# Farama-Foundation/Gymnasium

Hardware: AMD Instinct MI355X
Metric: env-steps/sec at num_envs=65536 (1/2/4/8 MI355X) vs CPU AsyncVectorEnv (higher is better)
Workload: dtype f64

## Files before the change

### gymnasium_amd/csrc/classic_kernels.h

```cpp
#ifndef MI355ENV_CLASSIC_KERNELS_H
#define MI355ENV_CLASSIC_KERNELS_H
#include "lane_step.h"
#include "wrappers_internal.h"

namespace {

MI_DEV double clip_to(double v, int flags, double lo, double hi) {
    if (flags & 1) v = v < lo ? lo : v;
    if (flags & 2) v = v > hi ? hi : v;
    return v;
}
__host__ __device__ inline bool epi_reduces(const EpiDev &e) { return (e.obs_on && e.obs_update) || (e.ret_on && e.ret_update); }

template <int NC>
MI_DEV void block_sum_columns(double (&v)[NC], double (*sh)[kEpiCols]) {
    const int wave = threadIdx.x >> 6, lane = threadIdx.x & 63;
#pragma unroll
    for (int k = 0; k < NC; k++) {
#pragma unroll
        for (int off = 32; off > 0; off >>= 1) v[k] += __shfl_xor(v[k], off, 64);
    }
    __syncthreads();
    if (lane == 0) {
#pragma unroll
        for (int k = 0; k < NC; k++) sh[wave][k] = v[k];
    }
    __syncthreads();
    if (threadIdx.x < NC) {
        double t = 0;
#pragma unroll
        for (int w = 0; w < kBlock / 64; w++) t += sh[w][threadIdx.x];
        v[0] = t;
    }
}

template <class E>
MI_DEV void epilogue_phase1(const EpiDev &e, int i, bool valid, const float *obs, double &reward, bool terminated) {
    constexpr int OBS = E::OBS, NC = 2 * OBS + 3;
    static_assert(OBS <= kEpiObsMax, "epilogue rows are sized for the classic-control observations");
    double v[NC];
#pragma unroll
    for (int k = 0; k < NC; k++) v[k] = 0;
    if (valid) {
        double r = clip_to(reward, e.clip_pre, e.pre_lo, e.pre_hi);
        if (e.ret_on) {
            const bool pd = e.prev_done[i] != 0, active = e.same_step || !pd;
            float a = e.acc[i];
            if (active) {
                const float g = a * e.gamma;
                a = (float)((double)g * (terminated ? 0.0 : 1.0) + r);
                e.acc[i] = a;
            }
            if (e.ret_update && active) {
                const double d = (double)a - e.ret_mean[0];
                v[2 * OBS] = d, v[2 * OBS + 1] = d * d, v[2 * OBS + 2] = 1.0;
            }
        } else {
            r = clip_to(r, e.clip_post, e.post_lo, e.post_hi);
        }
        reward = r;
        if (e.obs_on && e.obs_update) {
#pragma unroll
            for (int c = 0; c < OBS; c++) {
                const double d = (double)obs[c] - e.obs_mean[c];
                v[c] = d, v[OBS + c] = d * d;
            }
        }
    }
    if (!epi_reduces(e)) return;
    __shared__ double sh[kBlock / 64][kEpiCols];
    block_sum_columns<NC>(v, sh);
    if (threadIdx.x < NC) e.partial[(size_t)blockIdx.x * kEpiCols + threadIdx.x] = v[0];
}

template <int OBS>
MI_DEV void epilogue_statistics(const EpiDev &e, int N, bool fold, double (*sh)[kEpiCols], double *st) {
    constexpr int NC = 2 * OBS + 3;
    if (threadIdx.x < OBS && e.obs_on) st[threadIdx.x] = e.obs_mean[threadIdx.x], st[OBS + threadIdx.x] = e.obs_var[threadIdx.x];
    if (threadIdx.x == 64) {
        st[2 * OBS] = e.ret_on ? e.ret_var[0] : 1.0, st[2 * OBS + 1] = e.ret_on ? e.ret_mean[0] : 0.0;
        st[2 * OBS + 2] = e.obs_on ? *e.obs_count : 0.0, st[2 * OBS + 3] = e.ret_on ? *e.ret_count : 0.0;
    }
    if (fold) {
        double v[NC];
// ... 349 lines not shown
            ar.request(at, d, i);
            ar.arrive(L.trig);
        }
        u128 astate = 0;
        if (SAMPLE) {
            if (as.lane_valid) {
                astate = make_u128(as.lane[i], as.lane[(size_t)d.N + i]);
            } else {
                astate = make_u128(as.state_hi, as.state_lo);
                uint32_t delta = (uint32_t)i + 1u;
                for (int j = 0; delta; j++, delta >>= 1)
                    if (delta & 1u) astate = as.pow2[j].mult * astate + as.pow2[j].plus;
            }
        }
        const size_t N = (size_t)d.N;
        ResetQueue<E> q;
        q.have = 0u;
        q.rng = load_rng(d, i);
        WrapLaneOf<E, MAXSKIP> sl;
        load_wrap_lane(w, i, sl);
        if constexpr (MAXSKIP) load_skip_lane(w, d, i, sl);
        for (int t = 0; t < T; t++) {
            typename E::Act a;
            if (SAMPLE) {
                a = action_of_state<E>(astate);
                astate = as.jump_n.mult * astate + as.jump_n.plus;
                if (io.actions_out) static_cast<typename E::Act *>(io.actions_out)[t * N + i] = a;
            } else {
                a = static_cast<const typename E::Act *>(io.actions_in)[t * N + i];
            }
            StepOut<E> o;
            if (MODE == MI_AUTORESET_SAME_STEP) {
#pragma unroll
                for (int k = 0; k < E::OBS; k++) o.final_obs[k] = 0.0f;
            }
            if constexpr (MAXSKIP) q.have = 0u;
            lane_step_wrapped<E, MODE, MAXSKIP>(d, w, sl, i, L, a, o, st, &q, nullptr);
            if (io.obs) store_row<E::OBS>(static_cast<float *>(io.obs) + (t * N + i) * E::OBS, o.obs);
            if (io.reward) io.reward[t * N + i] = o.reward;
            if (io.terminated) io.terminated[t * N + i] = o.terminated;
            if (io.truncated) io.truncated[t * N + i] = o.truncated;
            if (ex.ep_ret) ex.ep_ret[t * N + i] = o.ep_ret;
            if (ex.ep_len) ex.ep_len[t * N + i] = o.ep_len;
            if (MODE == MI_AUTORESET_SAME_STEP && ex.final_obs) store_row<E::OBS>(static_cast<float *>(ex.final_obs) + (t * N + i) * E::OBS, o.final_obs);
        }
        if constexpr (MAXSKIP) {
            int wi = i;
            hold_opaque(wi);
            store_lane<E>(d, wi, L);
            store_wrap_lane(w, wi, sl);
            sl.written = 1u;
            store_skip_lane(w, d, wi, sl);
            store_rng_state(d, wi, q.rng);
            if (SAMPLE && as.lane) as.lane[wi] = (uint64_t)(astate >> 64), as.lane[N + wi] = (uint64_t)astate;
        } else {
            store_lane<E>(d, i, L);
            store_wrap_lane(w, i, sl);
            if (q.have) {
#pragma unroll
                for (int k = 0; k < E::NDRAWS; k++) q.rng.unstep();
            }
            store_rng_state(d, i, q.rng);
            if (SAMPLE && as.lane) as.lane[i] = (uint64_t)(astate >> 64), as.lane[N + i] = (uint64_t)astate;
        }
    }
    block_accumulate(d, st);
}

constexpr int kDuoBlock = 2 * kBlock;
template <class E>
struct DuoTraits {
#ifdef MI_DUO_CHUNK_OVERRIDE
    static constexpr int CHUNK = MI_DUO_CHUNK_OVERRIDE;
#else
    static constexpr int CHUNK = E::DUO_CHUNK;
#endif
};

template <class E, class = void>
struct HasRareHook : std::false_type {};
template <class E>
struct HasRareHook<E, std::void_t<decltype(E::RARE_HOOK)>> : std::integral_constant<bool, E::RARE_HOOK> {};

template <class E>
MI_DEV void duo_env_step(const DevEnv &d, Lane<E> &L, typename E::Act a, ResetQueue<E> &q, float obs[E::OBS], double &reward, uint32_t &bits) {
    const bool resetting = (L.flags & kNeedsReset) != 0;
    const bool refill = resetting && !q.have;
    constexpr bool HOOK = HasRareHook<E>::value && !E::SPLIT_TERMINAL && !E::AUX_REWARD;
    if (!HOOK && __builtin_expect(refill, 0)) q.refill();
    const double (&rs)[E::S] = q.rs;
    const uint32_t rflags = ResetQueue<E>::reset_flags(L.flags & ~kNeedsReset);
    double rew;
    bool te;
    uint32_t sflags = L.flags;
    if constexpr (E::SPLIT_TERMINAL) {
        E::integrate(L.s, sflags, a, L.trig);
#pragma unroll
        for (int k = 0; k < E::S; k++) L.s[k] = resetting ? rs[k] : L.s[k];
        E::obs(L.s, sflags, obs, L.trig);
        E::terminal_after_obs(L.s, L.trig, rew, te);
    } else if constexpr (E::AUX_REWARD) {
        E::advance(L.s, a, d.P, L.trig);
        rew = 0.0, te = false;
    } else if constexpr (HOOK) {
        E::step_hooked(L.s, sflags, a, d.P, rew, te, L.trig, refill, [&]() __attribute__((always_inline)) {
            if (refill) q.refill();
        });
    } else {
        E::step(L.s, sflags, a, d.P, rew, te, L.trig);
    }
    const uint32_t elapsed = L.elapsed + 1u;
    const bool tr = d.max_steps > 0 && (int)elapsed >= d.max_steps;
    const bool done = !resetting && (te || tr);
    if constexpr (!E::SPLIT_TERMINAL) {
#pragma unroll
        for (int k = 0; k < E::S; k++) L.s[k] = resetting ? rs[k] : L.s[k];
    }
    L.flags = resetting ? rflags : (done ? (sflags | kNeedsReset) : sflags);
    L.elapsed = resetting ? 0u : elapsed;
    q.have = resetting ? 0u : q.have;
    if constexpr (!E::SPLIT_TERMINAL) E::obs(L.s, L.flags, obs, L.trig);
    reward = resetting ? 0.0 : rew;
    bits = (resetting ? 4u : 0u) | ((!resetting && te) ? 1u : 0u) | ((!resetting && tr) ? 2u : 0u);
}

template <class E>
MI_DEV void duo_env_step_state(const DevEnv &d, Lane<E> &L, typename E::Act a, ResetQueue<E> &q, double *w64, float *w32) {
    static_assert(!E::SPLIT_TERMINAL, "the split terminal test belongs to the observation, which this role does not take");
    const bool resetting = (L.flags & kNeedsReset) != 0;
    if (__builtin_expect(resetting && !q.have, 0)) q.refill();
    const double (&rs)[E::S] = q.rs;
    const uint32_t rflags = ResetQueue<E>::reset_flags(L.flags & ~kNeedsReset);
    double rew;
    bool te;
    uint32_t sflags = L.flags;
    E::step(L.s, sflags, a, d.P, rew, te, L.trig);
    const uint32_t elapsed = L.elapsed + 1u;
    const bool tr = d.max_steps > 0 && (int)elapsed >= d.max_steps;
    const bool done = !resetting && (te || tr);
#pragma unroll
    for (int k = 0; k < E::S; k++) L.s[k] = resetting ? rs[k] : L.s[k];
    L.flags = resetting ? rflags : (done ? (sflags | kNeedsReset) : sflags);
    L.elapsed = resetting ? 0u : elapsed;
    q.have = resetting ? 0u : q.have;
    E::aux_pack(L.s, w64, w32);
}

template <class E>
__global__ __launch_bounds__(kDuoBlock) void rollout_duo_kernel(DevEnv d, RolloutPtrs io, ActionStream as, int T) {
    typedef typename E::Act Act;
    constexpr int ROLES = 2;
    constexpr int C = DuoTraits<E>::CHUNK;
    typedef Act ActLds;
    constexpr bool ACT_AHEAD = E::DUO_ACT_AHEAD;
    __shared__ ActLds sh_act[2][C + (ACT_AHEAD ? 1 : 0)][kBlock];
    constexpr bool DERIVE = E::AUX_DERIVES_FLAGS;
    static_assert(!DERIVE || E::REWARD_FROM_TERMINATED, "an aux role that derives the flags also derives the reward from them");
    constexpr int NF64 = E::AUX_F64 > 0 ? E::AUX_F64 : 1, NF32 = E::AUX_F32 > 0 ? E::AUX_F32 : 1;
    __shared__ double sh_w64[DERIVE ? 2 : 1][DERIVE ? C : 1][DERIVE ? kBlock : 1][NF64];
    __shared__ float sh_w32[(DERIVE && E::AUX_F32 > 0) ? 2 : 1][(DERIVE && E::AUX_F32 > 0) ? C : 1][(DERIVE && E::AUX_F32 > 0) ? kBlock : 1][NF32];
    __shared__ float sh_obs[DERIVE ? 1 : 2][DERIVE ? 1 : C][DERIVE ? 1 : kBlock][E::OBS];
    constexpr bool AUXREW = E::AUX_REWARD;
    constexpr bool REW_OF_ACT = E::AUX_REWARD_OF_ACTION;
    constexpr bool PASS_REWARD = !E::REWARD_FROM_TERMINATED && !AUXREW && !REW_OF_ACT;
    __shared__ double sh_pre[AUXREW ? 2 : 1][AUXREW ? C : 1][AUXREW ? kBlock : 1][E::AUX_PRE];
    __shared__ double sh_rew[PASS_REWARD ? 2 : 1][PASS_REWARD ? C : 1][kBlock];
    typedef typename std::conditional<E::REWARD_FROM_TERMINATED && E::OBS == 4, uint32_t, uint8_t>::type MI_DUO_FLAG_T;
    __shared__ MI_DUO_FLAG_T sh_bits[DERIVE ? 1 : 2][DERIVE ? 1 : C][DERIVE ? 1 : kBlock];
    __shared__ uint64_t sh_c[4][kBlock / 64];
    __shared__ double sh_r[kBlock / 64];
#ifdef MI_DUO_TIMING
    const unsigned long long t_begin = __builtin_readcyclecounter();
#endif
    tables_init<E>();
    const int role = threadIdx.x / kBlock;
    const bool is_env = role == 0, is_policy = role == 1, is_book = role == ROLES - 1;
    const int slot = threadIdx.x & (kBlock - 1);
    const int i = blockIdx.x * kBlock + slot;
    const bool active = i < d.N;
    const size_t N = (size_t)d.N;
    LaneStats st = {0u, 0u, 0u, 0ull, 0.0};
    Lane<E> L;
    ResetQueue<E> q;
    u128 astate = 0;
    double ep_ret = 0.0;
    int32_t ep_len = 0, ep_len_start = 0;
    uint32_t n_term = 0;
    uint32_t start_flags = 0;
    uint32_t aux_elapsed = 0, aux_needs_reset = 0;
    if (active) {
        if (is_env) {
            load_lane<E>(d, i, L);
            q.have = 0u;
            q.rng = load_rng(d, i);
        }
        if (is_book) {
            ep_ret = d.ep_ret[i], ep_len = d.ep_len[i];
            const uint32_t meta0 = d.meta[i];
            start_flags = meta0 >> kFlagShift;
            aux_elapsed = meta0 & kElapsedMask, aux_needs_reset = start_flags & kNeedsReset;
            ep_len_start = (start_flags & kNeedsReset) ? 0 : ep_len;
        }
        if (is_policy) {
            if (as.lane_valid) {
                astate = make_u128(as.lane[i], as.lane[N + i]);
            } else {
                astate = make_u128(as.state_hi, as.state_lo);
                uint32_t delta = (uint32_t)i + 1u;
                for (int j = 0; delta; j++, delta >>= 1)
                    if (delta & 1u) astate = as.pow2[j].mult * astate + as.pow2[j].plus;
            }
        }
    }
    const int chunks = T / C;
#ifdef MI_DUO_TIMING
    unsigned long long t_work = 0, t_wait = 0, t_wait0 = 0, t_mark = __builtin_readcyclecounter();
    const unsigned long long t_prologue = t_mark - t_begin;
#endif
    auto phase = [&](auto env_tag, const int p) __attribute__((always_inline)) {
        constexpr bool ENV = decltype(env_tag)::value;
        if (active) {
            if constexpr (ENV) {
                const int c = p - 1;
                if (c >= 0 && c < chunks) {
                    const int buf = c & 1;
                    constexpr bool REFILL_PER_CHUNK = kRefillPeriod % C == 0;
                    if (REFILL_PER_CHUNK && ((c * C) & (kRefillPeriod - 1)) == 0 && !q.have) q.refill();
                    ActLds a_next = sh_act[buf][0][slot];
#ifdef MI_DUO_ENV_UNROLL
#pragma unroll MI_DUO_ENV_UNROLL
#else
#pragma unroll 1
#endif
                    for (int k = 0; k < C; k++) {
                        const int t = c * C + k;
                        if (!REFILL_PER_CHUNK && (t & (kRefillPeriod - 1)) == 0 && !q.have) q.refill();
                        const Act a_k = ACT_AHEAD ? (Act)a_next : (Act)sh_act[buf][k][slot];
                        if (ACT_AHEAD) a_next = sh_act[buf][k + 1][slot];
                        if constexpr (DERIVE) {
                            double w64[NF64];
                            float w32[NF32];
                            duo_env_step_state<E>(d, L, a_k, q, w64, w32);
#pragma unroll
                            for (int j = 0; j < E::AUX_F64; j++) sh_w64[buf][k][slot][j] = w64[j];
#pragma unroll
                            for (int j = 0; j < E::AUX_F32; j++) sh_w32[buf][k][slot][j] = w32[j];
                        } else {
                            float o[E::OBS];
                            double rew;
                            uint32_t bits;
                            uint32_t pre_pending = 0u;
                            if constexpr (AUXREW) {
                                double pre[E::AUX_PRE];
                                pre_pending = E::aux_pre(L.s, pre);
#pragma unroll
                                for (int j = 0; j < E::AUX_PRE; j++) sh_pre[buf][k][slot][j] = pre[j];
                            }
                            duo_env_step<E>(d, L, a_k, q, o, rew, bits);
                            if constexpr (AUXREW && E::AUX_PRE_SQUARES > 0) bits |= pre_pending << 3;
#pragma unroll
                            for (int j = 0; j < E::OBS; j++) sh_obs[buf][k][slot][j] = o[j];
                            if constexpr (PASS_REWARD) sh_rew[buf][k][slot] = rew;
                            sh_bits[buf][k][slot] = (MI_DUO_FLAG_T)bits;
                        }
                    }
                }
            } else {
                const int c = p - 2;
                if (is_book && c >= 0) {
                    const int buf = c & 1;
                    if constexpr (AUXREW && E::AUX_PRE_SQUARES > 0) {
                        static_assert(E::AUX_PRE_SQUARES * C <= 32 && E::AUX_PRE_SQUARES <= 4 && sizeof(MI_DUO_FLAG_T) == 1, "pending bits: one word per chunk, bits 3 .. 6 of the flag byte");
                        uint32_t pend = 0u;
#pragma unroll
                        for (int k = 0; k < C; k++)
                            pend |= (((uint32_t)sh_bits[buf][k][slot] >> 3) & ((1u << E::AUX_PRE_SQUARES) - 1u)) << (E::AUX_PRE_SQUARES * k);
#pragma nounroll
                        while (pend) {
                            const int idx = __builtin_ctz(pend);
                            double *x = &sh_pre[buf][idx / E::AUX_PRE_SQUARES][slot][idx % E::AUX_PRE_SQUARES];
                            *x = E::aux_square(*x);
                            pend &= pend - 1u;
                        }
                    }
                    if constexpr (AUXREW) {
                        if constexpr (E::AUX_ACT_SQUARE) {
                            static_assert(C <= 32 && sizeof(ActLds) == sizeof(float), "one pending bit per step; the square takes the action's place");
                            uint32_t apend = 0u;
#pragma unroll
                            for (int k = 0; k < C; k++) {
                                const float u = E::act_square_arg((Act)sh_act[buf][k][slot]);
                                float h;
                                const bool plain = E::Math::sqf_is_plain(u, h);
                                sh_act[buf][k][slot] = (ActLds)(plain ? h : u);
                                apend |= plain ? 0u : 1u << k;
                            }
#pragma nounroll
                            while (apend) {
                                ActLds *x = &sh_act[buf][__builtin_ctz(apend)][slot];
                                *x = (ActLds)E::Math::sqf((float)*x);
                                apend &= apend - 1u;
                            }
                        }
                    }
#pragma unroll
                    for (int k = 0; k < C; k++) {
                        const size_t t = (size_t)c * C + k;
                        float o[E::OBS];
                        bool resetting, te, tr;
                        if constexpr (DERIVE) {
                            double w64[NF64];
                            float w32[NF32];
#pragma unroll
                            for (int j = 0; j < E::AUX_F64; j++) w64[j] = sh_w64[buf][k][slot][j];
#pragma unroll
                            for (int j = 0; j < E::AUX_F32; j++) w32[j] = sh_w32[buf][k][slot][j];
                            bool t0;
                            E::aux_unpack(w64, w32, d.P, o, t0);
                            resetting = aux_needs_reset != 0;
                            const uint32_t el = aux_elapsed + 1u;
                            te = !resetting && t0;
                            tr = !resetting && d.max_steps > 0 && (int)el >= d.max_steps;
                            aux_elapsed = resetting ? 0u : el;
                            aux_needs_reset = (te || tr) ? 1u : 0u;
                        } else {
#pragma unroll
                            for (int j = 0; j < E::OBS; j++) o[j] = sh_obs[buf][k][slot][j];
                            const uint32_t bits = sh_bits[buf][k][slot];
                            resetting = (bits & 4u) != 0, te = (bits & 1u) != 0, tr = (bits & 2u) != 0;
                        }
                        double rew;
                        const bool done = te || tr;
                        if constexpr (E::REWARD_FROM_TERMINATED) {
                            rew = resetting ? 0.0 : E::reward_from_terminated(te, d.P);
                            if constexpr (!DERIVE) ep_len = resetting ? 0 : ep_len + 1;
                            st.reset_steps += resetting ? 1u : 0u;
                            st.episodes += done ? 1u : 0u;
                            n_term += te ? 1u : 0u;
                        } else {
                            if constexpr (AUXREW) {
                                double pre[E::AUX_PRE];
#pragma unroll
                                for (int j = 0; j < E::AUX_PRE; j++) pre[j] = sh_pre[buf][k][slot][j];
                                if constexpr (E::AUX_ACT_SQUARE)
                                    rew = resetting ? 0.0 : E::aux_reward_squared(pre, (float)sh_act[buf][k][slot]);
                                else
                                    rew = resetting ? 0.0 : E::aux_reward(pre, (Act)sh_act[buf][k][slot]);
                            } else if constexpr (REW_OF_ACT) {
                                rew = resetting ? 0.0 : E::reward_of_action(te, (Act)sh_act[buf][k][slot]);
                            } else {
                                rew = sh_rew[buf][k][slot];
                            }
                            const double ret = ep_ret + rew;
                            const int32_t len = ep_len + 1;
                            ep_ret = resetting ? 0.0 : ret;
                            ep_len = resetting ? 0 : len;
                            st.reset_steps += resetting ? 1u : 0u;
                            st.env_steps += resetting ? 0u : 1u;
                            st.episodes += done ? 1u : 0u;
                            st.return_sum += done ? ret : 0.0;
                            st.length_sum += done ? (uint64_t)len : 0ull;
                        }
                        store_row<E::OBS>(static_cast<float *>(io.obs) + (t * N + i) * E::OBS, o);
                        io.reward[t * N + i] = rew;
                        io.terminated[t * N + i] = te;
                        io.truncated[t * N + i] = tr;
                    }
                }
                if (is_policy && p < chunks) {
                    const int buf = p & 1;
#pragma unroll
                    for (int k = 0; k < C; k++) {
                        const size_t t = (size_t)p * C + k;
                        const Act a = action_of_state<E>(astate);
                        astate = as.jump_n.mult * astate + as.jump_n.plus;
                        sh_act[buf][k][slot] = (ActLds)a;
                        static_cast<Act *>(io.actions_out)[t * N + i] = a;
                    }
                }
            }
        }
#ifdef MI_DUO_TIMING
        {
            const unsigned long long now = __builtin_readcyclecounter();
            t_work += now - t_mark, t_mark = now;
        }
#endif
        __syncthreads();
#ifdef MI_DUO_TIMING
        {
            const unsigned long long now = __builtin_readcyclecounter();
            if (p == 0) t_wait0 = now - t_mark;
            t_wait += now - t_mark, t_mark = now;
        }
#endif
    };
    if (__builtin_amdgcn_readfirstlane((int)is_env)) {
#pragma unroll 1
        for (int p = 0; p < chunks + 2; p++) phase(std::true_type(), p);
    } else {
#pragma unroll 1
        for (int p = 0; p < chunks + 2; p++) phase(std::false_type(), p);
    }
#ifdef MI_DUO_TIMING
    if (blockIdx.x == 7 && (threadIdx.x & 63) == 0)
        printf("duo timing: wave %d (role %d) prologue %llu work %llu wait-at-barrier %llu (phase 0: %llu) cycles over %d phases\n", (int)(threadIdx.x >> 6), role,
               t_prologue, t_work, t_wait, t_wait0, chunks + 2);
#endif
    if (active) {
        if (is_env) {
#pragma unroll
            for (int k = 0; k < E::S; k++) d.state[(size_t)k * d.N + i] = L.s[k];
            d.meta[i] = (L.elapsed & kElapsedMask) | (L.flags << kFlagShift);
            if (q.have) {
#pragma unroll
                for (int k = 0; k < E::NDRAWS; k++) q.rng.unstep();
            }
            store_rng_state(d, i, q.rng);
        } else if (is_book) {
            if constexpr (E::REWARD_FROM_TERMINATED) {
                const double r_n = E::reward_from_terminated(false, d.P), r_t = E::reward_from_terminated(true, d.P);
                bool last_done, last_te;
                if constexpr (DERIVE) {
                    double w64[NF64];
                    float w32[NF32], o[E::OBS];
#pragma unroll
                    for (int j = 0; j < E::AUX_F64; j++) w64[j] = sh_w64[((chunks > 0 ? chunks : 1) - 1) & 1][C - 1][slot][j];
#pragma unroll
                    for (int j = 0; j < E::AUX_F32; j++) w32[j] = sh_w32[((chunks > 0 ? chunks : 1) - 1) & 1][C - 1][slot][j];
                    bool t0;
                    E::aux_unpack(w64, w32, d.P, o, t0);
                    last_done = aux_needs_reset != 0, last_te = last_done && t0;
                } else {
                    const uint32_t last_bits = chunks > 0 ? (uint32_t)sh_bits[(chunks - 1) & 1][C - 1][slot] : ((start_flags & kNeedsReset) ? 2u : 0u);
                    last_done = (last_bits & 3u) != 0, last_te = (last_bits & 1u) != 0;
                }
                if (DERIVE && chunks > 0) ep_len = st.reset_steps ? (int32_t)aux_elapsed : ep_len + chunks * C;
                st.env_steps = (uint32_t)(chunks * C) - st.reset_steps;
                st.length_sum = (uint64_t)((int64_t)st.env_steps + (int64_t)ep_len_start - (last_done ? (int64_t)0 : (int64_t)ep_len));
                st.return_sum = r_n * (double)((int64_t)st.length_sum - (int64_t)n_term) + r_t * (double)n_term;
                st.return_sum = st.episodes ? st.return_sum : 0.0;
                ep_ret = (last_done && last_te) ? r_n * (double)(ep_len - 1) + r_t : r_n * (double)ep_len;
                if (chunks == 0) ep_ret = d.ep_ret[i];
            }
            d.ep_ret[i] = ep_ret, d.ep_len[i] = ep_len;
        }
        if (is_policy && as.lane) {
            int w = i;
            hold_opaque(w);
            as.lane[w] = (uint64_t)(astate >> 64), as.lane[N + w] = (uint64_t)astate;
        }
    }
    const int wave = slot >> 6, lane = threadIdx.x & 63;
    if (is_book) {
        const uint32_t c0 = wave_sum(st.env_steps), c1 = wave_sum(st.reset_steps), c2 = wave_sum(st.episodes);
        const uint64_t c3 = c2 ? wave_sum(st.length_sum) : 0;
        const double r = c2 ? wave_sum(st.return_sum) : 0.0;
        if (lane == 0) sh_c[0][wave] = c0, sh_c[1][wave] = c1, sh_c[2][wave] = c2, sh_c[3][wave] = c3, sh_r[wave] = r;
    }
    __syncthreads();
    if (threadIdx.x < 4) {
        uint64_t t = 0;
#pragma unroll
        for (int w = 0; w < kBlock / 64; w++) t += sh_c[threadIdx.x][w];
        if (t) d.blk_count[(size_t)blockIdx.x * 4 + threadIdx.x] += t;
    } else if (threadIdx.x == 64) {
        double t = 0.0;
#pragma unroll
        for (int w = 0; w < kBlock / 64; w++) t += sh_r[w];
        if (t != 0.0) d.blk_ret[blockIdx.x] += t;
    }
}

MI_DEV u128 shared_advance(const SharedRng &sr, u128 state, uint64_t n) {
    for (int j = 0; n; j++, n >>= 1)
        if (n & 1ull) state = sr.pow2[j].mult * state + sr.pow2[j].plus;
    return state;
}
MI_DEV void shared_block_bases(const SharedRng &sr, uint64_t first, uint64_t stride, uint64_t (*sh)[2]) {
    if (threadIdx.x < 4) {
        const u128 s = shared_advance(sr, make_u128(sr.words[0], sr.words[1]), first + (uint64_t)threadIdx.x * stride);
        sh[threadIdx.x][0] = (uint64_t)(s >> 64), sh[threadIdx.x][1] = (uint64_t)s;
    }
}
MI_DEV double shared_draw_from(const SharedRng &sr, const uint64_t (*sh)[2], int c, uint32_t offset) {
    Pcg64 g;
    g.state = shared_advance(sr, make_u128(sh[c][0], sh[c][1]), offset), g.inc = make_u128(sr.words[2], sr.words[3]);
    return g.next_double();
}

template <class E>
__global__ __launch_bounds__(kBlock) void shared_validate_kernel(DevEnv d, const typename E::Act *actions, SharedRng sr) {
    const int i = blockIdx.x * kBlock + threadIdx.x;
    if (i < d.N && !E::valid(actions[i])) {
        *d.error = kErrInvalidAction;
        sr.words[7] = 1;
    }
}

__global__ __launch_bounds__(kBlock) void shared_scan_kernel(SharedRng sr, int grid, uint64_t fixed_draws) {
    __shared__ uint32_t wave_total[kBlock / 64];
    if (!fixed_draws && sr.words[7]) return;
    const int per = (grid + kBlock - 1) / kBlock, lo = threadIdx.x * per, hi = min(grid, lo + per);
    const int lane = threadIdx.x & 63, wave = threadIdx.x >> 6;
    uint32_t sum = 0;
    if (!fixed_draws)
        for (int b = lo; b < hi; b++) sum += sr.blk_done[b];
    uint32_t incl = sum;
#pragma unroll
    for (int o = 1; o < 64; o <<= 1) {
        const uint32_t up = (uint32_t)__shfl_up((int)incl, o, 64);
        if (lane >= o) incl += up;
    }
    if (lane == 63) wave_total[wave] = incl;
    __syncthreads();
    uint32_t before = 0, total = 0;
#pragma unroll
// ... 143 lines not shown
```

### gymnasium_amd/csrc/envs_classic.h

```cpp
#pragma once
#include <hip/hip_runtime.h>
#include <stdint.h>

#include "../../include/mi355env.h"
#include "pcg64_dev.h"
#include "pow_exact.h"
#include "sincos_exact.h"

namespace mi {

#define MI_DEV __device__ __forceinline__

constexpr double kPi = 3.141592653589793;

enum : uint32_t { kNeedsReset = 1u, kStateF32 = 2u };

static __shared__ double g_trig6[660 + 18];
static __shared__ double g_pow_log[384];
static __shared__ uint64_t g_pow_exp[256];
static __shared__ double g_powf_log2[32];
static __shared__ uint64_t g_powf_exp2[32];

struct TwoPi {
    static constexpr double value = 2 * kPi;
};
#ifndef MI_HOT_TRIG
#define MI_HOT_TRIG true
#endif

struct SharedDivisor {
    double b, r;
    SharedDivisor() = default;
    MI_DEV explicit SharedDivisor(double divisor) : b(divisor) {
        const double r0 = __builtin_amdgcn_rcp(divisor);
        const double e0 = __builtin_fma(-divisor, r0, 1.0);
        const double r1 = __builtin_fma(r0, e0, r0);
        const double e1 = __builtin_fma(-divisor, r1, 1.0);
        r = __builtin_fma(r1, e1, r1);
    }
    MI_DEV double under(double a) const {
        const double q0 = a * r;
        const double e = __builtin_fma(-b, q0, a);
        return __builtin_amdgcn_div_fixup(__builtin_fma(e, r, q0), b, a);
    }
    static MI_DEV bool ordinary(double a) { return (((uint32_t)(mi_sincos::bits(a) >> 32) & 0x7fffffffu) - 0x20000000u) < 0x40000000u; }
};
template <bool KASM>
struct ExactMathT {
    static constexpr bool EXACT = true;
    template <bool POW, bool POWF>
    static MI_DEV void init() {
        for (int e = threadIdx.x; e < 110; e += blockDim.x) mi_sincos::expand6(mi_sincos::kTable, g_trig6, e);
        if (threadIdx.x == 0) mi_sincos::fill_hot(g_trig6);
        if (POW) {
            for (int k = threadIdx.x; k < 384; k += blockDim.x) g_pow_log[k] = mi_pow::kLogTab[k];
            for (int k = threadIdx.x; k < 256; k += blockDim.x) g_pow_exp[k] = mi_pow::kExpTab[k];
        }
        if (POWF) {
            for (int k = threadIdx.x; k < 32; k += blockDim.x) g_powf_log2[k] = mi_pow::kLog2fTab[k], g_powf_exp2[k] = mi_pow::kExp2fTab[k];
        }
        __syncthreads();
    }
    static constexpr bool HOT = MI_HOT_TRIG;
    static MI_DEV double sin(double x) { return mi_sincos::sin_bf<false, KASM, HOT>(g_trig6, x); }
    static MI_DEV double cos(double x) { return mi_sincos::cos_bf<false, KASM, HOT>(g_trig6, x); }
    static MI_DEV void sincos(double x, double &s, double &c) { mi_sincos::sincos_bf<false, true, KASM>(g_trig6, x, s, c); }
    static MI_DEV void sincos_main_unchecked(double x, double &s, double &c) { mi_sincos::sincos_main<KASM>(g_trig6, x, s, c); }
    static MI_DEV bool in_main_range(double x) { return ((uint32_t)(mi_sincos::bits(x) >> 32) & 0x7fffffffu) < 0x3feb6000u; }
    static MI_DEV void sincos_spread(double x, double &s, double &c) { mi_sincos::sincos_bf<false, false, KASM, HOT>(g_trig6, x, s, c); }
    static MI_DEV double sin_bounded(double x) { return mi_sincos::sin_bf<true, KASM, HOT>(g_trig6, x); }
    static MI_DEV double cos_bounded(double x) { return mi_sincos::cos_bf<true, KASM, HOT>(g_trig6, x); }
    static MI_DEV void sincos_bounded(double x, double &s, double &c) { mi_sincos::sincos_bf<true, false, KASM, HOT>(g_trig6, x, s, c); }
    static MI_DEV double cos_bounded_literals(double x) { return mi_sincos::cos_bf<true, KASM>(g_trig6, x); }
    static MI_DEV double fmod_2pi(double x) { return mi_sincos::fmod_const(x, TwoPi()); }
    static MI_DEV double sq(double x) { return mi_pow::square<KASM>(g_pow_log, g_pow_exp, x); }
    static MI_DEV float sqf(float x) { return mi_pow::squaref<KASM>(g_powf_log2, g_powf_exp2, x); }
    static MI_DEV void sq3(double a, double b, double c, double &ra, double &rb, double &rc) { mi_pow::square3<KASM>(g_pow_log, g_pow_exp, a, b, c, ra, rb, rc); }
    static MI_DEV void sq2(double a, double b, double &ra, double &rb) { mi_pow::square2<KASM>(g_pow_log, g_pow_exp, a, b, ra, rb); }
    static MI_DEV bool sq_is_plain(double x, double &hi) { return mi_pow::square_is_plain(x, hi); }
    static MI_DEV bool sqf_is_plain(float x, float &hi) { return mi_pow::squaref_is_plain(x, hi); }
};
typedef ExactMathT<true> ExactMath;
typedef ExactMathT<false> ExactMathBuiltinFma;
struct FastMath {
    static constexpr bool EXACT = false;
    template <bool POW, bool POWF>
    static MI_DEV void init() {}
    static MI_DEV double sin(double x) { return ::sin(x); }
    static MI_DEV double cos(double x) { return ::cos(x); }
    static MI_DEV void sincos(double x, double &sn, double &cs) {
        if (__builtin_expect(!(fabs(x) <= 0.7853981633974483), 0)) {
            ::sincos(x, &sn, &cs);
            return;
        }
        auto fma_k = [](double a, double b, double c) { return mi_sincos::fma_k<true>(a, b, c); };
        const double z = x * x;
        const double S1 = -1.66666666666666324348e-01, S2 = 8.33333333332248946124e-03, S3 = -1.98412698298579493134e-04,
                     S4 = 2.75573137070700676789e-06, S5 = -2.50507602534068634195e-08, S6 = 1.58969099521155010221e-10;
        const double C1 = 4.16666666666666019037e-02, C2 = -1.38888888888741095749e-03, C3 = 2.48015872894767294178e-05,
                     C4 = -2.75573143513906633035e-07, C5 = 2.08757232129817482790e-09, C6 = -1.13596475577881948265e-11;
        double rs = fma_k(z, S6, S5);
        rs = fma_k(z, rs, S4), rs = fma_k(z, rs, S3), rs = fma_k(z, rs, S2), rs = fma_k(z, rs, S1);
        sn = fma(z * x, rs, x);
        double rc = fma_k(z, C6, C5);
        rc = fma_k(z, rc, C4), rc = fma_k(z, rc, C3), rc = fma_k(z, rc, C2), rc = fma_k(z, rc, C1);
        const double hz = 0.5 * z;
        const double w = 1.0 - hz;
        cs = w + (((1.0 - w) - hz) + z * (z * rc));
    }
    static MI_DEV void sincos_spread(double x, double &s, double &c) { ::sincos(x, &s, &c); }
    static MI_DEV double sin_bounded(double x) { return ::sin(x); }
    static MI_DEV double cos_bounded(double x) { return ::cos(x); }
    static MI_DEV double cos_bounded_literals(double x) { return ::cos(x); }
    static MI_DEV void sincos_bounded(double x, double &s, double &c) { ::sincos(x, &s, &c); }
    static MI_DEV double fmod_2pi(double x) { return ::fmod(x, 2 * kPi); }
    static MI_DEV double sq(double x) { return x * x; }
    static MI_DEV float sqf(float x) { return x * x; }
    static MI_DEV void sq3(double a, double b, double c, double &ra, double &rb, double &rc) { ra = a * a, rb = b * b, rc = c * c; }
    static MI_DEV void sq2(double a, double b, double &ra, double &rb) { ra = a * a, rb = b * b; }
    static MI_DEV bool sq_is_plain(double x, double &hi) { return hi = x * x, true; }
    static MI_DEV bool sqf_is_plain(float x, float &hi) { return hi = x * x, true; }
};
template <class E>
MI_DEV void tables_init() {
    E::Math::template init<E::USES_POW, E::USES_POWF>();
}

template <class C>
MI_DEV double div_by_constant(double x, C) {
    constexpr double c = C::value, r = 1.0 / C::value;
    const double q = x * r;
    const double q2 = fma(fma(-q, c, x), r, q);
    const double ax = fabs(x);
    if (__builtin_expect(!(ax <= 1e300 && ax >= 1e-300), 0)) return x / c;
    return q2;
}

template <class C>
MI_DEV double div_by_constant_unchecked(double x, C) {
    constexpr double c = C::value, r = 1.0 / C::value;
    const double q = x * r;
    return fma(fma(-q, c, x), r, q);
}
MI_DEV bool div_by_constant_in_range(double x) {
    const double ax = fabs(x);
    return (ax <= 1e300) & (ax >= 1e-300);
}

MI_DEV double div_unscaled(double x, double y) {
    const double r0 = __builtin_amdgcn_rcp(y);
    const double r1 = __builtin_fma(r0, __builtin_fma(-y, r0, 1.0), r0);
    const double r = __builtin_fma(r1, __builtin_fma(-y, r1, 1.0), r1);
    const double q0 = x * r;
    return __builtin_fma(__builtin_fma(-y, q0, x), r, q0);
}

struct EnvParams {
    double p[16];
};

struct NoTrig {};
struct PendulumTrig {
    double sn, cs;
    bool ok;
};
struct AcrobotTrig {
    double s1, c1, s2, c2;
    bool ok;
};
MI_DEV void trig_invalidate(NoTrig &) {}
MI_DEV void trig_invalidate(PendulumTrig &t) { t.ok = false; }
MI_DEV void trig_invalidate(AcrobotTrig &t) { t.ok = false; }

struct ActF32 {
    typedef float T;
    static constexpr int KIND = MI_F32;
};
struct ActF64 {
    typedef double T;
    static constexpr int KIND = MI_F64;
};
struct ActF64Weak {
    typedef double T;
    static constexpr int KIND = MI_F64_WEAK;
};

struct CartPoleTotalMass {
    static constexpr double value = 0.1 + 1.0;
};
template <class M>
struct CartPoleT {
    typedef M Math;
    static constexpr bool SPLIT_TERMINAL = false;
    static constexpr bool USES_POW = false, USES_POWF = false;
    typedef CartPoleTotalMass TotalMass;
    static constexpr int S = 4, OBS = 4, N_ACTIONS = 2;
    static constexpr bool DISCRETE = true;
    static constexpr int ACT_KIND = MI_I64;
    static constexpr int ROLLOUT_UNROLL = 1;
    static constexpr bool DUO_ROLLOUT = true;
    static constexpr int DUO_CHUNK = 8;
    static constexpr bool DUO_ACT_AHEAD = false;
    static constexpr bool REWARD_FROM_TERMINATED = true;
    static MI_DEV double reward_from_terminated(bool terminated, const EnvParams &P) {
        const bool sutton_barto = P.p[0] != 0.0;
        return terminated ? (sutton_barto ? -1.0 : 1.0) : (sutton_barto ? 0.0 : 1.0);
    }
    static constexpr bool AUX_DERIVES_FLAGS = false;
    static constexpr bool AUX_REWARD = false;
    static constexpr bool AUX_REWARD_OF_ACTION = false;
    template <class A>
    static MI_DEV double reward_of_action(bool, A) { return 0.0; }
    static constexpr int AUX_PRE = 1;
    static constexpr int AUX_PRE_SQUARES = 0;
    static MI_DEV uint32_t aux_pre(const double *, double *) { return 0u; }
    static MI_DEV double aux_square(double x) { return x; }
    static MI_DEV double aux_reward(const double *, int64_t) { return 0.0; }
    static constexpr int AUX_F64 = 2, AUX_F32 = 2;
    static MI_DEV void aux_pack(const double s[S], double w64[AUX_F64], float w32[AUX_F32]) {
        w64[0] = s[0], w64[1] = s[2], w32[0] = (float)s[1], w32[1] = (float)s[3];
    }
    static MI_DEV void aux_unpack(const double w64[AUX_F64], const float w32[AUX_F32], const EnvParams &, float o[OBS], bool &terminated) {
        const double theta_threshold = 12 * 2 * kPi / 360, x_threshold = 2.4;
        const double x = w64[0], theta = w64[1];
        o[0] = (float)x, o[1] = w32[0], o[2] = (float)theta, o[3] = w32[1];
        terminated = x < -x_threshold || x > x_threshold || theta < -theta_threshold || theta > theta_threshold;
    }
    typedef int64_t Act;

    static MI_DEV void default_bounds(double &b0, double &b1) { b0 = -0.05, b1 = 0.05; }

    static constexpr int NDRAWS = 4;
    static MI_DEV void reset_u(const double u[NDRAWS], double s[S], uint32_t &flags, double b0, double b1) {
        const double range = b1 - b0;
#pragma unroll
        for (int k = 0; k < S; k++) s[k] = b0 + range * u[k];
        (void)flags;
    }
    typedef NoTrig Trig;
    static MI_DEV void obs(const double s[S], uint32_t, float o[OBS], Trig &) {
#pragma unroll
        for (int k = 0; k < OBS; k++) o[k] = (float)s[k];
    }
    static MI_DEV bool valid(Act a) { return a >= 0 && a < N_ACTIONS; }
    static MI_DEV Act sample(double u) { return (Act)(u * 2.0); }
    static constexpr bool SAMPLE_FROM_BITS = true;
    static MI_DEV Act sample_bits(uint64_t bits) { return (Act)(bits >> 63); }
    static MI_DEV Act sample_state(uint64_t hi, uint64_t lo) {
        const unsigned rot = (unsigned)(hi >> 58);
        return (Act)(((hi ^ lo) >> ((rot + 63u) & 63u)) & 1ull);
    }

    struct Accel {
        double thetaacc, xacc;
    };
    static __device__ __attribute__((noinline)) Accel general_accel(double theta, double theta_dot, double force) {
        const double gravity = 9.8, masspole = 0.1, length = 0.5;
        const double polemass_length = masspole * length;
        double sintheta, costheta;
        M::sincos(theta, sintheta, costheta);
        const double temp = div_by_constant(force + polemass_length * (theta_dot * theta_dot) * sintheta, TotalMass());
        Accel r;
        r.thetaacc = (gravity * sintheta - costheta * temp) /
                     (length * (4.0 / 3.0 - div_by_constant(masspole * (costheta * costheta), TotalMass())));
        r.xacc = temp - div_by_constant(polemass_length * r.thetaacc * costheta, TotalMass());
        return r;
    }
    static MI_DEV void step(double s[S], uint32_t &f, Act action, const EnvParams &P, double &reward, bool &terminated, Trig &t) {
        step_hooked(s, f, action, P, reward, terminated, t, false, [] {});
    }
    static constexpr bool RARE_HOOK = true;
    template <class F>
    static MI_DEV void step_hooked(double s[S], uint32_t &, Act action, const EnvParams &P, double &reward, bool &terminated, Trig &, bool extra, F &&rare) {
        const double gravity = 9.8, masspole = 0.1, length = 0.5, force_mag = 10.0, tau = 0.02;
        const double polemass_length = masspole * length;
        const double theta_threshold = 12 * 2 * kPi / 360;
        const double x_threshold = 2.4;
        double x = s[0], x_dot = s[1], theta = s[2], theta_dot = s[3];
        const double force = action == 1 ? force_mag : -force_mag;
        double costheta, sintheta;
        double temp, thetaacc, xacc;
        if constexpr (M::EXACT) {
            const bool main_range = M::in_main_range(theta);
            M::sincos_main_unchecked(theta, sintheta, costheta);
            const double t1 = force + polemass_length * (theta_dot * theta_dot) * sintheta;
// ... 787 lines not shown
```

Baseline: 131.7 billion.

## Pack CartPole episode state into a single word and unroll the env loop

Adds an episode word that packs the pending-reset flag, elapsed count and reset-queue 'have' bit into one 32-bit register, so the env role's per-step bookkeeping shrinks to a few integer ops. Enables it for CartPole by default. The same change raises CartPole's env-loop unroll to 8 and replaces the main-range bit test with a fabs compare. An optional raw-flags mode, off by default, moves reset masking to the book role. Risks are more register pressure from the unroll and subtle changes to the reset and truncation semantics.

```diff
diff --git a/gymnasium_amd/csrc/classic_kernels.h b/gymnasium_amd/csrc/classic_kernels.h
--- a/gymnasium_amd/csrc/classic_kernels.h
+++ b/gymnasium_amd/csrc/classic_kernels.h
@@ -1,5 +1,6 @@
 #ifndef MI355ENV_CLASSIC_KERNELS_H
 #define MI355ENV_CLASSIC_KERNELS_H
+#include "episode_word.h"
 #include "lane_step.h"
 #include "wrappers_internal.h"
 
@@ -515,6 +516,21 @@
 template <class E>
 struct HasRareHook<E, std::void_t<decltype(E::RARE_HOOK)>> : std::integral_constant<bool, E::RARE_HOOK> {};
 
+template <class E, class = void>
+struct DuoEpisodeWord : std::false_type {};
+template <class E>
+struct DuoEpisodeWord<E, std::void_t<decltype(E::DUO_EPISODE_WORD)>> : std::integral_constant<bool, E::DUO_EPISODE_WORD> {};
+template <class E, class = void>
+struct DuoRawFlags : std::false_type {};
+template <class E>
+struct DuoRawFlags<E, std::void_t<decltype(E::DUO_RAW_FLAGS)>> : std::integral_constant<bool, E::DUO_RAW_FLAGS> {};
+template <class E, class = void>
+struct DuoEnvUnroll : std::integral_constant<int, 1> {};
+template <class E>
+struct DuoEnvUnroll<E, std::void_t<decltype(E::DUO_ENV_UNROLL)>> : std::integral_constant<int, E::DUO_ENV_UNROLL> {};
+static_assert(mi_episode_word::kMetaFlagShift == kFlagShift && mi_episode_word::kMetaElapsedMask == kElapsedMask && mi_episode_word::kMetaNeedsReset == kNeedsReset,
+              "episode_word.h restates the layout of `meta`");
+
 template <class E>
 MI_DEV void duo_env_step(const DevEnv &d, Lane<E> &L, typename E::Act a, ResetQueue<E> &q, float obs[E::OBS], double &reward, uint32_t &bits) {
     const bool resetting = (L.flags & kNeedsReset) != 0;
@@ -555,6 +571,36 @@
     if constexpr (!E::SPLIT_TERMINAL) E::obs(L.s, L.flags, obs, L.trig);
     reward = resetting ? 0.0 : rew;
     bits = (resetting ? 4u : 0u) | ((!resetting && te) ? 1u : 0u) | ((!resetting && tr) ? 2u : 0u);
+}
+
+template <class E, bool RAW>
+MI_DEV void duo_env_step_word(const DevEnv &d, Lane<E> &L, typename E::Act a, ResetQueue<E> &q, uint32_t &ew, const int32_t thr, float obs[E::OBS], double &reward, uint32_t &bits) {
+    namespace W = mi_episode_word;
+    static_assert(!E::SPLIT_TERMINAL && !E::AUX_REWARD && !E::AUX_DERIVES_FLAGS, "measured for the plain env role only (CartPole)");
+    const bool resetting = W::resetting(ew);
+    const bool refill = W::refill(ew);
+    constexpr bool HOOK = HasRareHook<E>::value;
+    if (!HOOK && __builtin_expect(refill, 0)) q.refill();
+    const double (&rs)[E::S] = q.rs;
+    const uint32_t rflags = ResetQueue<E>::reset_flags(L.flags);
+    double rew;
+    bool te;
+    uint32_t sflags = L.flags;
+    if constexpr (HOOK) {
+        E::step_hooked(L.s, sflags, a, d.P, rew, te, L.trig, refill, [&]() __attribute__((always_inline)) {
+            if (refill) q.refill();
+        });
+    } else {
+        E::step(L.s, sflags, a, d.P, rew, te, L.trig);
+    }
+    const bool tr = W::truncated(ew, thr);
+#pragma unroll
+    for (int k = 0; k < E::S; k++) L.s[k] = resetting ? rs[k] : L.s[k];
+    L.flags = resetting ? rflags : sflags;
+    ew = W::advance(ew, te || tr);
+    E::obs(L.s, L.flags, obs, L.trig);
+    reward = resetting ? 0.0 : rew;
+    bits = RAW ? W::flag_bits(te, tr) : ((resetting ? 4u : 0u) | W::flag_bits(!resetting && te, tr));
 }
 
 template <class E>
@@ -586,6 +632,8 @@
     constexpr int C = DuoTraits<E>::CHUNK;
     typedef Act ActLds;
     constexpr bool ACT_AHEAD = E::DUO_ACT_AHEAD;
+    constexpr bool WORD = DuoEpisodeWord<E>::value, RAW = DuoRawFlags<E>::value;
+    static_assert(!RAW || WORD, "the unmasked flags are duo_env_step_word's");
     __shared__ ActLds sh_act[2][C + (ACT_AHEAD ? 1 : 0)][kBlock];
     constexpr bool DERIVE = E::AUX_DERIVES_FLAGS;
     static_assert(!DERIVE || E::REWARD_FROM_TERMINATED, "an aux role that derives the flags also derives the reward from them");
@@ -615,6 +663,8 @@
     LaneStats st = {0u, 0u, 0u, 0ull, 0.0};
     Lane<E> L;
     ResetQueue<E> q;
+    uint32_t ew = 0u;
+    const int32_t ew_thr = WORD ? mi_episode_word::truncation_threshold(d.max_steps) : 0;
     u128 astate = 0;
     double ep_ret = 0.0;
     int32_t ep_len = 0, ep_len_start = 0;
@@ -626,6 +676,10 @@
             load_lane<E>(d, i, L);
             q.have = 0u;
             q.rng = load_rng(d, i);
+            if constexpr (WORD) {
+                ew = mi_episode_word::encode((L.elapsed & kElapsedMask) | (L.flags << kFlagShift), 0u);
+                L.flags &= ~kNeedsReset;
+            }
         }
         if (is_book) {
             ep_ret = d.ep_ret[i], ep_len = d.ep_len[i];
@@ -658,16 +712,24 @@
                 if (c >= 0 && c < chunks) {
                     const int buf = c & 1;
                     constexpr bool REFILL_PER_CHUNK = kRefillPeriod % C == 0;
-                    if (REFILL_PER_CHUNK && ((c * C) & (kRefillPeriod - 1)) == 0 && !q.have) q.refill();
+                    if constexpr (WORD) {
+                        if (REFILL_PER_CHUNK && ((c * C) & (kRefillPeriod - 1)) == 0 && !mi_episode_word::have(ew)) q.refill(), ew = mi_episode_word::with_have(ew);
+                    } else {
+                        if (REFILL_PER_CHUNK && ((c * C) & (kRefillPeriod - 1)) == 0 && !q.have) q.refill();
+                    }
                     ActLds a_next = sh_act[buf][0][slot];
 #ifdef MI_DUO_ENV_UNROLL
 #pragma unroll MI_DUO_ENV_UNROLL
 #else
-#pragma unroll 1
+#pragma unroll(DuoEnvUnroll<E>::value)
 #endif
                     for (int k = 0; k < C; k++) {
                         const int t = c * C + k;
-                        if (!REFILL_PER_CHUNK && (t & (kRefillPeriod - 1)) == 0 && !q.have) q.refill();
+                        if constexpr (WORD) {
+                            if (!REFILL_PER_CHUNK && (t & (kRefillPeriod - 1)) == 0 && !mi_episode_word::have(ew)) q.refill(), ew = mi_episode_word::with_have(ew);
+                        } else {
+                            if (!REFILL_PER_CHUNK && (t & (kRefillPeriod - 1)) == 0 && !q.have) q.refill();
+                        }
                         const Act a_k = ACT_AHEAD ? (Act)a_next : (Act)sh_act[buf][k][slot];
                         if (ACT_AHEAD) a_next = sh_act[buf][k + 1][slot];
                         if constexpr (DERIVE) {
@@ -689,7 +751,10 @@
 #pragma unroll
                                 for (int j = 0; j < E::AUX_PRE; j++) sh_pre[buf][k][slot][j] = pre[j];
                             }
-                            duo_env_step<E>(d, L, a_k, q, o, rew, bits);
+                            if constexpr (WORD)
+                                duo_env_step_word<E, RAW>(d, L, a_k, q, ew, ew_thr, o, rew, bits);
+                            else
+                                duo_env_step<E>(d, L, a_k, q, o, rew, bits);
                             if constexpr (AUXREW && E::AUX_PRE_SQUARES > 0) bits |= pre_pending << 3;
 #pragma unroll
                             for (int j = 0; j < E::OBS; j++) sh_obs[buf][k][slot][j] = o[j];
@@ -760,7 +825,14 @@
 #pragma unroll
                             for (int j = 0; j < E::OBS; j++) o[j] = sh_obs[buf][k][slot][j];
                             const uint32_t bits = sh_bits[buf][k][slot];
-                            resetting = (bits & 4u) != 0, te = (bits & 1u) != 0, tr = (bits & 2u) != 0;
+                            if constexpr (RAW) {
+                                resetting = aux_needs_reset != 0;
+                                const uint32_t eff = mi_episode_word::effective_flags(aux_needs_reset, bits);
+                                te = (eff & 1u) != 0, tr = (eff & 2u) != 0;
+                                aux_needs_reset = eff;
+                            } else {
+                                resetting = (bits & 4u) != 0, te = (bits & 1u) != 0, tr = (bits & 2u) != 0;
+                            }
                         }
                         double rew;
                         const bool done = te || tr;
@@ -844,7 +916,8 @@
         if (is_env) {
 #pragma unroll
             for (int k = 0; k < E::S; k++) d.state[(size_t)k * d.N + i] = L.s[k];
-            d.meta[i] = (L.elapsed & kElapsedMask) | (L.flags << kFlagShift);
+            if constexpr (WORD) d.meta[i] = mi_episode_word::decode_meta(ew, L.flags), q.have = mi_episode_word::have(ew);
+            else d.meta[i] = (L.elapsed & kElapsedMask) | (L.flags << kFlagShift);
             if (q.have) {
 #pragma unroll
                 for (int k = 0; k < E::NDRAWS; k++) q.rng.unstep();
@@ -865,7 +938,7 @@
                     E::aux_unpack(w64, w32, d.P, o, t0);
                     last_done = aux_needs_reset != 0, last_te = last_done && t0;
                 } else {
-                    const uint32_t last_bits = chunks > 0 ? (uint32_t)sh_bits[(chunks - 1) & 1][C - 1][slot] : ((start_flags & kNeedsReset) ? 2u : 0u);
+                    const uint32_t last_bits = chunks > 0 ? (RAW ? aux_needs_reset : (uint32_t)sh_bits[(chunks - 1) & 1][C - 1][slot]) : ((start_flags & kNeedsReset) ? 2u : 0u);
                     last_done = (last_bits & 3u) != 0, last_te = (last_bits & 1u) != 0;
                 }
                 if (DERIVE && chunks > 0) ep_len = st.reset_steps ? (int32_t)aux_elapsed : ep_len + chunks * C;
diff --git a/gymnasium_amd/csrc/envs_classic.h b/gymnasium_amd/csrc/envs_classic.h
--- a/gymnasium_amd/csrc/envs_classic.h
+++ b/gymnasium_amd/csrc/envs_classic.h
@@ -26,6 +26,18 @@
 };
 #ifndef MI_HOT_TRIG
 #define MI_HOT_TRIG true
+#endif
+#ifndef MI_MAIN_RANGE_FABS
+#define MI_MAIN_RANGE_FABS 1
+#endif
+#ifndef MI_CP_EPISODE_WORD
+#define MI_CP_EPISODE_WORD 1
+#endif
+#ifndef MI_CP_RAW_FLAGS
+#define MI_CP_RAW_FLAGS 0
+#endif
+#ifndef MI_CP_ENV_UNROLL
+#define MI_CP_ENV_UNROLL 8
 #endif
 
 struct SharedDivisor {
@@ -66,7 +78,11 @@
     static MI_DEV double cos(double x) { return mi_sincos::cos_bf<false, KASM, HOT>(g_trig6, x); }
     static MI_DEV void sincos(double x, double &s, double &c) { mi_sincos::sincos_bf<false, true, KASM>(g_trig6, x, s, c); }
     static MI_DEV void sincos_main_unchecked(double x, double &s, double &c) { mi_sincos::sincos_main<KASM>(g_trig6, x, s, c); }
+#if MI_MAIN_RANGE_FABS
+    static MI_DEV bool in_main_range(double x) { return __builtin_fabs(x) < 0.85546875; }
+#else
     static MI_DEV bool in_main_range(double x) { return ((uint32_t)(mi_sincos::bits(x) >> 32) & 0x7fffffffu) < 0x3feb6000u; }
+#endif
     static MI_DEV void sincos_spread(double x, double &s, double &c) { mi_sincos::sincos_bf<false, false, KASM, HOT>(g_trig6, x, s, c); }
     static MI_DEV double sin_bounded(double x) { return mi_sincos::sin_bf<true, KASM, HOT>(g_trig6, x); }
     static MI_DEV double cos_bounded(double x) { return mi_sincos::cos_bf<true, KASM, HOT>(g_trig6, x); }
@@ -201,6 +217,9 @@
     static constexpr bool DUO_ROLLOUT = true;
     static constexpr int DUO_CHUNK = 8;
     static constexpr bool DUO_ACT_AHEAD = false;
+    static constexpr bool DUO_EPISODE_WORD = MI_CP_EPISODE_WORD;
+    static constexpr bool DUO_RAW_FLAGS = DUO_EPISODE_WORD && MI_CP_RAW_FLAGS;
+    static constexpr int DUO_ENV_UNROLL = MI_CP_ENV_UNROLL;
     static constexpr bool REWARD_FROM_TERMINATED = true;
     static MI_DEV double reward_from_terminated(bool terminated, const EnvParams &P) {
         const bool sutton_barto = P.p[0] != 0.0;
diff --git a/gymnasium_amd/csrc/episode_word.h b/gymnasium_amd/csrc/episode_word.h
--- /dev/null
+++ b/gymnasium_amd/csrc/episode_word.h
@@ -0,0 +1,40 @@
+#ifndef MI355ENV_EPISODE_WORD_H
+#define MI355ENV_EPISODE_WORD_H
+#include <stdint.h>
+
+#if defined(__HIPCC__) || defined(__CUDACC__)
+#define MI_EW_FN __host__ __device__ __forceinline__
+#else
+#define MI_EW_FN inline
+#endif
+
+namespace mi_episode_word {
+
+constexpr uint32_t kPending = 0x80000000u, kHave = 1u;
+constexpr uint32_t kMetaFlagShift = 30, kMetaElapsedMask = (1u << kMetaFlagShift) - 1u, kMetaNeedsReset = 1u;
+
+MI_EW_FN uint32_t encode(uint32_t meta, uint32_t have) {
+    return (((meta >> kMetaFlagShift) & kMetaNeedsReset) ? kPending : 0u) | ((meta & kMetaElapsedMask) << 1) | (have ? kHave : 0u);
+}
+MI_EW_FN uint32_t decode_meta(uint32_t w, uint32_t other_flags) {
+    return ((w >> 1) & kMetaElapsedMask) | (((other_flags & ~kMetaNeedsReset) | (w >> 31)) << kMetaFlagShift);
+}
+MI_EW_FN uint32_t have(uint32_t w) { return w & kHave; }
+MI_EW_FN uint32_t with_have(uint32_t w) { return w | kHave; }
+
+MI_EW_FN int32_t truncation_threshold(int max_steps) { return max_steps > 0 ? (int32_t)(2u * (uint32_t)(max_steps < (1 << 30) ? max_steps : (1 << 30) - 1)) : INT32_MAX; }
+
+MI_EW_FN bool resetting(uint32_t w) { return (int32_t)w < 0; }
+MI_EW_FN bool refill(uint32_t w) { return (w & (kPending | kHave)) == kPending; }
+MI_EW_FN bool truncated(uint32_t w, int32_t threshold) { return (int32_t)(w + 2u) >= threshold; }
+MI_EW_FN bool done(uint32_t w, bool terminated, int32_t threshold) { return !resetting(w) && (terminated || truncated(w, threshold)); }
+
+MI_EW_FN uint32_t advance(uint32_t w, bool ended) { return resetting(w) ? 0u : ((w + 2u) | (ended ? kPending : 0u)); }
+MI_EW_FN uint32_t step(uint32_t w, bool terminated, int32_t threshold) { return advance(w, terminated || truncated(w, threshold)); }
+
+MI_EW_FN uint32_t flag_bits(bool terminated, bool truncated) { return (terminated ? 1u : 0u) | (truncated ? 2u : 0u); }
+MI_EW_FN uint32_t raw_flags(uint32_t w, bool terminated, int32_t threshold) { return flag_bits(terminated, truncated(w, threshold)); }
+MI_EW_FN uint32_t effective_flags(uint32_t pending, uint32_t raw) { return pending ? 0u : raw; }
+
+}
+#endif
```

Result: faster. 134.1 billion (median of 6 runs) (+1.8%).
